# GadGadGad/Convolutional-KAN-for-Image-Classification

Measured on AMD Instinct MI355X. Metric: images/sec fwd+bwd KAN-VGG11 3x32x32 bs=256/GPU, higher is better.
Workload: dtype f32

## Files before the change

### convolutional-kan-for-image-classification_amd/_lib.py

```python
from __future__ import annotations

import ctypes as C
import os
from typing import Optional

_HERE = os.path.dirname(os.path.abspath(__file__))
LIB_PATH = os.environ.get("KANCONV_LIB") or os.path.join(_HERE, "libkanconv.so")

KAN_MAX_PLANES = 16
KAN_MAX_TABLE = 32
KAN_FP_WORDS = 192
BASIS_BSPLINE, BASIS_RBF, BASIS_CHEBY, BASIS_POLY, BASIS_FOURIER, BASIS_RELU, BASIS_GRAM = 0, 1, 2, 3, 4, 5, 6
ACT_NONE, ACT_IDENTITY, ACT_GELU, ACT_SILU, ACT_RELU, ACT_TANH, ACT_SIGMOID, ACT_GELU_TANH = -1, 0, 1, 2, 3, 4, 5, 6
ORDER_QUAD_FWD, ORDER_ROWBLK8_FWD, ORDER_QUAD_BWD_DATA, ORDER_FWD_WEIGHT_SIDE, ORDER_POS8_BWD_DATA = 1, 2, 4, 8, 16


class KanGeom(C.Structure):
    _fields_ = [(n, C.c_int) for n in ("B", "C", "H", "W", "O", "Ho", "Wo", "kh", "kw", "sh", "sw", "ph", "pw", "dh", "dw", "groups")] + \
               [("x_bstride", C.c_longlong), ("y_bstride", C.c_longlong)]


class KanBasis(C.Structure):
    _fields_ = [("kind", C.c_int), ("n_basis", C.c_int), ("order", C.c_int), ("act", C.c_int),
                ("p0", C.c_float), ("p1", C.c_float), ("table", C.c_float * KAN_MAX_TABLE), ("chan_table", C.c_void_p)]


class KanPlan(C.Structure):
    _fields_ = [(n, C.c_int) for n in ("P", "K", "IPC", "KC", "Kpad", "Opad", "fwd_splits", "bwd_data_splits", "bwd_weight_splits",
                                          "fwd_target", "bwd_data_target", "bwd_weight_target", "x_pm_wanted", "dz_pm_wanted", "bwd_weight_expanded", "row_blocks", "e_pm_wanted", "fwd_expanded", "fwd_halo", "bwd_weight_halo",
                                          "fwd_band", "bwd_weight_band")] + \
               [(n, C.c_longlong) for n in ("packed_weight_bytes", "bwd_data_weight_bytes", "fwd_slab_elems", "bwd_data_slab_elems",
                                            "bwd_weight_slab_elems", "e_pm_elems")]


class KanNormRoute(C.Structure):
    _fields_ = [(n, C.c_int) for n in ("kernel", "G", "EPL", "PPI", "NT", "pool", "lds", "held", "blocks", "strided")]

# ... 6 lines not shown
    _fields_ = [(n, C.c_int) for n in ("B", "C", "H", "W", "O", "Ho", "Wo", "kh", "kw", "sh", "sw", "ph", "pw", "dh", "dw", "wavelet")] + \
               [("x_bstride", C.c_longlong), ("u_bstride", C.c_longlong)]


class KanWavRoute(C.Structure):
    _fields_ = [(n, C.c_int) for n in ("TH", "TW", "NIMG", "RH", "RW", "tiles_h", "tiles_w", "fwd_shrunk", "fwd_nimg_cut", "fwd_lds_bytes", "fwd_fits",
                                       "fwd_blocks", "bwd_input_kernel", "bwd_input_blocks", "params_kernel", "passes", "chunks", "BH", "NI", "RU",
                                       "CU", "XP", "UP", "bands", "items", "items_per_chunk", "lds_bytes", "px_per_chunk")]


WAV_BI_TAPS9, WAV_BI_STRIDE1, WAV_BI_STRIDED = 0, 1, 2
WAV_PAR_TILED, WAV_PAR_PIXEL = 0, 1


WAVELETS = {"mexican_hat": 0, "morlet": 1, "dog": 2, "meyer": 3, "shannon": 4}

_P, _I, _LL, _F, _D = C.c_void_p, C.c_int, C.c_longlong, C.c_float, C.c_double
_GP, _BP = C.POINTER(KanGeom), C.POINTER(KanBasis)
SIGNATURES = {
    "kan_version": (C.c_char_p, []),
    "kan_last_error": (C.c_char_p, []),
    "kan_plan": (_I, [_GP, _BP, C.POINTER(KanPlan)]),
    "kan_tile_orders": (_I, [_GP, _BP]),
    "kan_pack_weights": (_I, [_P, _P, _P, _P, _GP, _BP, _P]),
    "kan_pack_weights_iod": (_I, [_P, _P, _P, _GP, _BP, _P]),
    "kan_pack_cacheable": (_I, [_GP, _BP]),
    "kan_pack_weights_cached": (_I, [_P, _P, _P, _P, _GP, _BP, _P, _I, _I, _I, _P]),
    "kan_conv_fwd": (_I, [_P, _P, _P, _P, _GP, _BP, _P, _P]),
    "kan_position_major": (_I, [_P, _P, _I, _I, _I, _LL, _P]),
    "kan_conv_bwd_data": (_I, [_P, _P, _P, _P, _P, _P, _GP, _BP, _P, _P]),
    "kan_conv_bwd_data_params": (_I, [_P, _P, _P, _P, _P, _P, _P, _GP, _BP, _P, _P]),
    "kan_conv_bwd_weight": (_I, [_P, _P, _P, _P, _GP, _BP, _P, _P, _P]),
    "kan_position_major_expanded": (_I, [_P, _P, _GP, _BP, _P]),
    "kan_conv_fwd_expanded": (_I, [_P, _P, _P, _GP, _BP, _P]),
    "kan_conv_fwd_expanded_order": (_I, [_P, _P, _P, _GP, _BP, _P, _I]),
    "kan_conv_bwd_weight_expanded": (_I, [_P, _P, _P, _GP, _BP, _P]),
    "kan_unpack_wgrad": (_I, [_P, _P, _P, _GP, _BP, _P]),
    "kan_unpack_wgrad_iod": (_I, [_P, _P, _GP, _BP, _P]),
    "kan_slab_reduce": (_I, [_P, _I, _LL, _P, _I, _I, _I, _LL, _P]),
    "kan_instnorm_prelu_fwd": (_I, [_P, _I, _LL, _P, _P, _P, _P, _P, _P, _P, _I, _I, _I, _LL, _F, _I, _P]),
    "kan_instnorm_prelu_bwd": (_I, [_P, _P, _P, _P, _P, _P, _P, _P, _P, _P, _P, _I, _I, _I, _LL, _I, _P]),
    "kan_instnorm_prelu_pool_fwd": (_I, [_P, _I, _LL, _P, _P, _P, _P, _P, _P, _P, _P, _I, _I, _I, _I, _LL, _F, _I, _P]),
    "kan_instnorm_prelu_pool_bwd": (_I, [_P, _P, _P, _P, _P, _P, _P, _P, _P, _P, _P, _P, _I, _I, _I, _I, _LL, _I, _P]),
    "kan_instnorm_prelu_poolk_fwd": (_I, [_P, _I, _LL, _P, _P, _P, _P, _P, _P, _P, _P, _I, _I, _I, _I, _LL, _F, _I, _I, _I, _P]),
    "kan_instnorm_prelu_poolk_bwd": (_I, [_P, _P, _P, _P, _P, _P, _P, _P, _P, _P, _P, _P, _I, _I, _I, _I, _LL, _I, _I, _I, _P]),
    "kan_norm_route": (_I, [_I, _I, _I, _I, _I, _LL, _I, _LL, _I, _I, _I, _I, C.POINTER(KanNormRoute)]),
# ... 75 lines not shown
```

### convolutional-kan-for-image-classification_amd/csrc/kan_internal.h

```cpp
#pragma once
#include <type_traits>
#include "kanconv.h"

int kan_fail_msg(const char* fmt, const char* a);
int kan_raise_lds_limit(const void* kernel, int bytes);

enum : int {
    FAST_GENERIC = 0,
    FAST_BSPLINE_SILU = 1,
    FAST_BSPLINE_GELU = 2,
    FAST_RBF8 = 3,
    FAST_CHEBY5 = 4,
    FAST_CHEBY4 = 5,
    FAST_POLY4 = 6,
    FAST_POLY3 = 7,
    FAST_RBF5 = 8,
    FAST_RELU8 = 9,
    FAST_GRAM4 = 10,
    FAST_POLY1 = 11,
    FAST_LAST = 11
};
enum : unsigned {
    ON_TAP_MAJOR = 1u << 0,
    ON_BIG_TILES = 1u << 1,
// ... 85 lines not shown
                               const KanBandCfg* cfg, int splits, long long slab_elems, void* stream);
int kan_band_fwd_launch(const float* x, const float* xn, const float* wp, float* z, const KanGeom* g, const KanBasis* b,
                        const KanBandCfg* cfg, int splits, long long slab_elems, void* stream);

constexpr int DW_T = 9;
constexpr int DW_MAX_TP = 96;

enum class Route { TAP_MAJOR, DW, BAND, HALO, EXPANDED };

struct FwdCfg { int TO, TP, tiles_o, tiles_p, chunks, splits, slots; };
struct BdCfg { int CH, tiles_c, tiles_p, n_ob, Opad32, chunks, splits; };
struct BwCfg { int TR, TO, tiles_r, tiles_o, chunks, splits, slots; };
struct BwHaloCfg { int R, nimg, spb, n_bands, tiles_r, tiles_o, splits, bands_per_split; };

struct ConvPlan {
    KanPlan pub;
    int fast;
    Route fwd, bwd_data, bwd_weight;
    bool pm_fwd, pm_bwd_data, pm_bwd_weight;
    bool rowblk_bwd_data;
    bool quad_fwd;
    bool quad_bd;
    bool pos8_bd;
    bool rowblk8_fwd;
    bool fwd_wq;
    bool pmdma_xcd, pm_lpt, pm_xcd;
    FwdCfg fc;
    BdCfg bd;
    BwCfg bw;
    BwHaloCfg bwh;
    KanBandCfg band;
};
int plan_conv(const KanGeom* g, const KanBasis* b, ConvPlan* cp);

int live_taps_out(const KanGeom* g, int hw);
int live_taps_in(const KanGeom* g, int hw);
int live_positions_for_tap(const KanGeom* g, int tap);
int balance_tiles(const int* weight, int n, unsigned short* idx);
```

### convolutional-kan-for-image-classification_amd/csrc/kan_plan.hip

```cpp
#include <hip/hip_runtime.h>
#include <cstdio>
#include <cstdlib>
#include <cstring>
#include "kanconv.h"
#include "kan_device.h"
#include "kan_common.h"
#include "kan_internal.h"

namespace {

int fail(const char* msg) { return kan_fail_msg("%s", msg); }

int check(const KanGeom* g, const KanBasis* b) {
    if (!g || !b) return fail("null geometry/basis");
    if (g->groups < 0 || g->groups > 65535) return fail("groups out of range");
    if (g->B <= 0 || g->C <= 0 || g->O <= 0 || g->H <= 0 || g->W <= 0 || g->Ho <= 0 || g->Wo <= 0) return fail("non-positive dimension");
    if (g->kh <= 0 || g->kw <= 0 || g->sh <= 0 || g->sw <= 0 || g->dh <= 0 || g->dw <= 0 || g->ph < 0 || g->pw < 0) return fail("bad conv parameters");
    if (g->kh > 255 || g->kw > 255 || g->C > 65535) return fail("kernel size / channel count out of supported range");
    if ((g->H + 2 * g->ph - g->dh * (g->kh - 1) - 1) / g->sh + 1 != g->Ho || (g->W + 2 * g->pw - g->dw * (g->kw - 1) - 1) / g->sw + 1 != g->Wo)
        return fail("Ho/Wo inconsistent with H/W, kernel, stride, padding, dilation");
    if ((long long)g->B * g->Ho * g->Wo >= (1ll << 31) || (long long)g->B * g->H * g->W >= (1ll << 31)) return fail("pixel count exceeds int32");
    if ((long long)g->B * g->x_bstride * 4 >= (1ll << 31) || (long long)g->B * g->y_bstride * 4 >= (1ll << 31))
        return fail("activation tensors must be smaller than 2 GiB (32-bit buffer offsets)");
    if (g->x_bstride < (long long)ngroups(g) * g->C * g->H * g->W || g->y_bstride < (long long)ngroups(g) * g->O * g->Ho * g->Wo)
// ... 179 lines not shown
}
BwHaloCfg bw_halo_cfg(const KanGeom* g, const KanPlan& pl) {
    BwHaloCfg c;
    c.R = g->W == 16 ? 4 : g->W;
    c.nimg = g->W == 4 ? 2 : 1;
    c.spb = c.nimg * c.R * g->W / 16;
    c.n_bands = g->B * (g->H / c.R) / c.nimg;
    c.tiles_r = ceil_div(pl.K, 128);
    c.tiles_o = pl.Opad / 128;
    const long long tiles = (long long)c.tiles_r * c.tiles_o * ngroups(g);
    const double slab_bytes = 4.0 * pl.K * pl.Opad * ngroups(g);
    int best = 1; double best_cost = -1;
    for (int sp = 1; sp <= c.n_bands && sp <= 1024; ++sp) {
        const int bps = ceil_div(c.n_bands, sp);
        if (ceil_div(c.n_bands, bps) != sp) continue;
        const long long rounds = (tiles * sp + 1023) / 1024;
        const double cost = (double)(rounds * (bps * c.spb + 6)) + sp * slab_cost_steps(slab_bytes);
        if (best_cost < 0 || cost < best_cost) { best_cost = cost; best = sp; }
    }
    c.splits = best;
    c.bands_per_split = ceil_div(c.n_bands, best);
    return c;
}
BwCfg bw_cfg(const KanGeom* g, const KanPlan& pl, bool big, bool pm_bw) {
    BwCfg c;
    c.TO = (big && !pm_bw) ? 256 : (pl.Opad % 128 == 0) ? 128 : 64;
    c.slots = c.TO == 256 ? 512 : 1024;
    c.TR = c.TO == 64 ? 256 : 128;
    c.tiles_r = ceil_div(pl.K, c.TR);
    c.tiles_o = pl.Opad / c.TO;
    c.chunks = ceil_div((long long)g->B * g->Ho * g->Wo, 16);
    c.splits = pick_splits((long long)c.tiles_r * c.tiles_o * ngroups(g), c.chunks, 16, 4.0 * pl.K * pl.Opad * ngroups(g), c.slots);
    return c;
}

bool dw_direct(const KanGeom* g, const KanBasis* b) {
    const bool off = tuning_off("KAN_DW");
    const int T = g->kh * g->kw, P = b->n_basis + (b->act != KAN_ACT_NONE);
    return !off && g->C == 1 && g->O <= 2 && T <= DW_T && T * P <= DW_MAX_TP;
}
int dw_weight_chunks(const KanGeom* g) {
    const long long total = (long long)g->B * g->Ho * g->Wo;
    int s = ceil_div(2048, ngroups(g));
    const int most = ceil_div(total, 256);
    if (s > most) s = most;
    if (s > 64) s = 64;
// ... 49 lines not shown
    for (int i = 0; i < n; ++i) { if (idx[i] >= n || seen[idx[i]]) return 0; seen[idx[i]] = true; }
    return n;
}

int plan_conv(const KanGeom* g, const KanBasis* b, ConvPlan* cp) {
    if (int rc = check(g, b)) return rc;
    ConvPlan& c = *cp;
    KanPlan* pl = &c.pub;
    const int T = g->kh * g->kw, G = ngroups(g), f = fast_variant(b);
    c.fast = f;
    const bool pm_shape = pmdma_fwd_shape(g, f);
    c.pm_fwd = want_pix_major(g, b, PM_FWD, pm_shape);
    c.pm_bwd_data = want_pix_major(g, b, PM_BWD_DATA, false);
    const bool want_pm_bw = want_pix_major(g, b, PM_BWD_WEIGHT, false);
    const bool dw = dw_direct(g, b);
    const bool halo = halo_fwd(g, b, f, c.pm_fwd);
    c.band.ok = c.band.bw_ok = 0;
    const bool band = band_fwd(g, b, f, dw, c.pm_fwd, halo, &c.band);
    const bool pmdma_fwd = pm_shape && c.pm_fwd;
    const bool pmdma_bw = pmdma_bwd_weight(g, b, f, want_pm_bw);
    const bool halo_bw = halo_bwd_weight(g, f, pmdma_bw);
    c.pm_bwd_weight = want_pm_bw && !halo_bw;
    const bool band_bw = band && c.band.bw_ok && !want_pm_bw && !tuning_off("KAN_BAND_BW");
    c.rowblk_bwd_data = rowblk_bwd_data(g, f, c.pm_bwd_data);
    c.pmdma_xcd = tuning_on("KAN_PMDMA_XCD");
    c.pm_lpt = !tuning_off("KAN_PM_LPT");
    c.pm_xcd = !tuning_off("KAN_PM_XCD");
    c.fwd = dw ? Route::DW : band ? Route::BAND : halo ? Route::HALO : pmdma_fwd ? Route::EXPANDED : Route::TAP_MAJOR;
    c.bwd_data = dw ? Route::DW : Route::TAP_MAJOR;
    c.bwd_weight = dw ? Route::DW : band_bw ? Route::BAND : halo_bw ? Route::HALO : pmdma_bw ? Route::EXPANDED : Route::TAP_MAJOR;
    pl->P = b->n_basis + (b->act != KAN_ACT_NONE);
    pl->K = g->C * T * pl->P;
    {
        int i18 = 18 / pl->P, i16 = 16 / pl->P;
        if (i18 > 4) i18 = 4;
        if (i16 > 4) i16 = 4;
        const bool use18 = (long long)i18 * pl->P * 16 > (long long)i16 * pl->P * 18;
        pl->KC = use18 ? 18 : 16;
        pl->IPC = use18 ? i18 : i16;
        if (pl->P >= 10 && pl->P <= 12) { pl->KC = 12; pl->IPC = 1; }
        if (halo) { pl->KC = 2 * pl->P; pl->IPC = 2; }
    }
    pl->Kpad = ceil_div(g->C * T, pl->IPC) * pl->KC;
    if (band) { pl->KC = c.band.NPLE; pl->IPC = c.band.NG; pl->Kpad = c.band.n_steps * c.band.NPLE; }
    pl->Opad = round_up(g->O, 64);
    pl->packed_weight_bytes = (long long)G * pl->Kpad * pl->Opad * 4;
// ... 64 lines not shown
```

### convolutional-kan-for-image-classification_amd/csrc/kanconv.hip

```cpp
#include <hip/hip_runtime.h>
#include <cstdio>
#include <cstdlib>
#include <cstring>
#include <cmath>
#include <cstdint>
#include <mutex>
#include <type_traits>
#include <vector>
#include "kanconv.h"
#include "kan_device.h"

#include "kan_common.h"
#include "kan_internal.h"

namespace {


thread_local char g_err[512] = "";
int fail(const char* fmt, const char* a = "") {
    snprintf(g_err, sizeof(g_err), fmt, a);
    return -1;
}
}
int kan_fail_msg(const char* fmt, const char* a) { return fail(fmt, a); }
// ... 1557 lines not shown
                acc[0][0] = MFMA32(fa[c_][0], fb[c_][0], acc[0][0]);
                acc[0][1] = MFMA32(fa[c_][0], fb[c_][1], acc[0][1]);
                acc[1][0] = MFMA32(fa[c_][1], fb[c_][0], acc[1][0]);
                acc[1][1] = MFMA32(fa[c_][1], fb[c_][1], acc[1][1]);
            }
#undef KAN_OFFA
#undef KAN_OFFB
        }
    }

    float* out = dwp + (size_t)blk.z * slab_elems;
#pragma unroll
    for (int mi = 0; mi < 2; ++mi)
#pragma unroll
        for (int r = 0; r < 16; ++r) {
            const int row = k0 + w_r * 64 + mi * 32 + mfma_row(r, lane);
            if (row >= Krows) continue;
#pragma unroll
            for (int ni = 0; ni < 2; ++ni) {
                const int o = o_tile0 + w_c * 64 + ni * 32 + (lane & 31);
                out[(size_t)row * Opad + o] = acc[mi][ni][r];
            }
        }
}

template <int KIND, int FAST>
__global__ __launch_bounds__(256) void k_expand_pm(const float* __restrict__ x, float* __restrict__ e_pm, DevBasis bs, int B, int CHW, int HW, int Cg,
                                                   long long bstride, float* __restrict__ dump) {
    __shared__ float tile[32][33];
    __shared__ float sTab[KAN_MAX_TABLE];
    const int e0 = blockIdx.x * 32, b0 = blockIdx.y * 32;
    const int tx = threadIdx.x & 31, ty = threadIdx.x >> 5;
    const int P = FAST ? fast_planes(FAST) : bs.P;
    if (threadIdx.x < KAN_MAX_TABLE) sTab[threadIdx.x] = bs.tab[threadIdx.x];
#pragma unroll
    for (int i = 0; i < 4; ++i) {
        const int b = b0 + ty + 8 * i, e = e0 + tx;
        tile[ty + 8 * i][tx] = (b < B && e < CHW) ? x[(size_t)b * bstride + e] : 0.f;
    }
    __syncthreads();
#pragma unroll
    for (int i = 0; i < 4; ++i) {
        const int e = e0 + ty + 8 * i, b = b0 + tx;
        if (e < CHW && b < B) {
            const float v = tile[tx][ty + 8 * i];
            stage_unit<KIND, FAST>(bs, sTab, true, v, v, e_pm + (size_t)e * P * B + b, B, dump + threadIdx.x, (e / HW) % Cg);
// ... 1246 lines not shown
        const int bx = c.tiles_c * 4, by = c.Opad32 / 32 * G;
        const long long nt = (long long)bx * by;
        const long long capd = fp ? 128 : 1024;
        dim3 gd((unsigned)(nt < capd ? nt : capd), 1, T);
        hipLaunchKernelGGL(k_pack_bwd_data, gd, dim3(256), 0, st, (const float*)wp, wd, q, c.CH, c.tiles_c, c.Opad32, wp_gs, bx, by, fp, fp_cur);
    }
    return launch_ok("pack");
}

int kan_pack_weights(const float* w_base, const float* w_basis, float* wp, float* wd, const KanGeom* g, const KanBasis* b, void* stream) {
    return pack_weights_impl(w_base, w_basis, wp, wd, g, b, nullptr, 0, stream);
}

int kan_pack_weights_iod(const float* coeffs, float* wp, float* wd, const KanGeom* g, const KanBasis* b, void* stream) {
    if (int rc = iod_scope(g, b)) return rc;
    return pack_weights_impl(nullptr, coeffs, wp, wd, g, b, nullptr, 0, stream, true);
}

int kan_tile_orders(const KanGeom* g, const KanBasis* b) {
    ConvPlan cp;
    if (plan_conv(g, b, &cp)) return 0;
    const bool halo = cp.fwd == Route::HALO;
    return (halo && cp.quad_fwd ? KAN_ORDER_QUAD_FWD : 0) | (halo && cp.rowblk8_fwd ? KAN_ORDER_ROWBLK8_FWD : 0) | (cp.quad_bd ? KAN_ORDER_QUAD_BWD_DATA : 0) |
           (cp.fwd_wq ? KAN_ORDER_FWD_WEIGHT_SIDE : 0) | (cp.pos8_bd ? KAN_ORDER_POS8_BWD_DATA : 0);
}

int kan_pack_cacheable(const KanGeom* g, const KanBasis* b) {
    ConvPlan cp;
    if (plan_conv(g, b, &cp)) return 0;
    if ((long long)g->O * g->C * (b->n_basis + 1) * g->kh * g->kw >= (1ll << 31)) return 0;
    return (!pack_needs_clear(g, cp.pub) && cp.fwd != Route::DW && ngroups(g) == 1) ? 1 : 0;
}

int kan_pack_weights_cached(const float* w_base, const float* w_basis, float* wp, float* wd, const KanGeom* g, const KanBasis* b,
                            unsigned long long* ring, int cur, int force, int sample_stride, void* stream) {
    static_assert(KAN_FP_WORDS == 3 * FP_LANES, "ring size");
    if (!ring || cur < 0 || cur > 2 || sample_stride < 1) return fail("bad fingerprint ring arguments");
    if (!kan_pack_cacheable(g, b)) return fail("cached packing is not offered for this geometry (kan_pack_cacheable)");
    const int hb = b->act != KAN_ACT_NONE;
    if ((hb && !w_base) || !w_basis) return fail("null weight pointer");
    if (((size_t)w_basis & 15) || (hb && ((size_t)w_base & 15))) return fail("cached packing needs 16-byte aligned weight tensors");
    const int T = g->kh * g->kw;
    const long long na = hb ? (long long)g->O * g->C * T : 0, nbs = (long long)g->O * g->C * b->n_basis * T;
    const long long groups4 = ((na + 3) / 4 + (nbs + 3) / 4 + sample_stride - 1) / sample_stride;
    long long blocks = (groups4 + 256 * 8 - 1) / (256 * 8); if (blocks > 4096) blocks = 4096; if (blocks < 1) blocks = 1;
    hipLaunchKernelGGL(k_fingerprint, dim3((unsigned)blocks), dim3(256), 0, (hipStream_t)stream, hb ? w_base : w_basis, (unsigned)na, w_basis,
                       (unsigned)nbs, (unsigned)sample_stride, ring, cur);
    if (int rc = launch_ok("fingerprint")) return rc;
    return pack_weights_impl(w_base, w_basis, wp, wd, g, b, force ? nullptr : ring, cur, stream);
}

static int unpack_wgrad_impl(const float* dwp, float* dw_base, float* dw_basis, const KanGeom* g, const KanBasis* b, void* stream, bool iod) {
    ConvPlan cp;
    if (int rc = plan_conv(g, b, &cp)) return rc;
    const KanPlan& pl = cp.pub;
    const int hb = b->act != KAN_ACT_NONE;
    if ((hb && !dw_base) || !dw_basis || !dwp) return fail("null weight-gradient pointer");
    hipStream_t st = (hipStream_t)stream;
    const int T = g->kh * g->kw, G = ngroups(g);
    const long long dwp_gs = (long long)(pl.bwd_weight_band ? pl.Kpad : pl.K) * pl.Opad;
    PackGeo q = pack_geo(g, b, cp, true);
    int n_slabs = pl.bwd_weight_splits;
    if (n_slabs >= 32) {
        hipLaunchKernelGGL(k_fold_slabs, dim3(ceil_div(pl.bwd_weight_slab_elems, 64)), dim3(256), 0, st, const_cast<float*>(dwp), n_slabs,
                           pl.bwd_weight_slab_elems, pl.bwd_weight_slab_elems);
        n_slabs = 1;
    }
    const int nb_base = hb ? ceil_div(g->C * T, UNPACK_TJ) : 0;
    dim3 grid(nb_base + ceil_div(g->C * b->n_basis * T, UNPACK_TJ), ceil_div(g->O, UNPACK_TO), G);
    if (iod) {
        const IodLaunch l = iod_launch(g, pl);
        hipLaunchKernelGGL(k_unpack_iod, dim3(l.blocks), dim3(256), 0, st, dwp, dw_basis, q, l.o_tiles, l.n_tiles, n_slabs, pl.bwd_weight_slab_elems,
                           iod_vec(dw_basis, dwp, g, b));
    } else {
        hipLaunchKernelGGL(k_unpack, grid, dim3(256), 0, st, dwp, dw_base, dw_basis, q, nb_base, n_slabs, pl.bwd_weight_slab_elems, dwp_gs);
    }
    return launch_ok("unpack");
}

int kan_unpack_wgrad(const float* dwp, float* dw_base, float* dw_basis, const KanGeom* g, const KanBasis* b, void* stream) {
    return unpack_wgrad_impl(dwp, dw_base, dw_basis, g, b, stream, false);
}

int kan_unpack_wgrad_iod(const float* dwp, float* dcoeffs, const KanGeom* g, const KanBasis* b, void* stream) {
    if (int rc = iod_scope(g, b)) return rc;
    return unpack_wgrad_impl(dwp, nullptr, dcoeffs, g, b, stream, true);
}

int kan_position_major(const float* src, float* dst, int B, int Cn, int HW, long long bstride, void* stream) {
    if (!src || !dst || B < 1 || Cn < 1 || HW < 1) return fail("bad position_major arguments");
    dim3 grid(ceil_div((long long)Cn * HW, 32), ceil_div(B, 32));
    hipLaunchKernelGGL(k_position_major, grid, dim3(256), 0, (hipStream_t)stream, src, dst, B, Cn * HW, bstride);
    return launch_ok("position_major");
}

int kan_conv_fwd(const float* x, const float* xn, const float* wp, float* z, const KanGeom* g, const KanBasis* b, const float* x_pm,
                 void* stream) {
    ConvPlan cp;
    if (int rc = plan_conv(g, b, &cp)) return rc;
    const KanPlan& pl = cp.pub;
    if (!x || !xn || !wp || !z) return fail("null tensor pointer");
    if ((b->kind == KAN_BASIS_RELU || b->kind == KAN_BASIS_GRAM) && !b->chan_table) return fail("ReLU / Gram bases need their device parameter table (chan_table)");
    hipStream_t st = (hipStream_t)stream;
    if (cp.fwd == Route::DW) {
// ... 198 lines not shown
    const int cps = dg.pix_major ? pl.bwd_weight_target : ceil_div(c.chunks, pl.bwd_weight_splits);
    if (x != xn && !fast_spec(cp.fast).xn_fwd)
        return fail("this basis / activation pair runs on single-input kernels: pass xn == x");
    auto launch = [&](auto kind, auto fast, auto wr, auto wc) {
        constexpr int WR = decltype(wr)::value, WC = decltype(wc)::value;
        hipLaunchKernelGGL((k_conv_bwd_weight<decltype(kind)::value, decltype(fast)::value, WR, WC>), grid, dim3(WR * WC * 64), 0, st, dz, x, xn, dwp,
                           dg, db, pl.K, pl.Opad, c.chunks, cps, pl.bwd_weight_slab_elems, x_bytes, dz_bytes, c.tiles_o);
    };
    auto tiles = [&](auto kind, auto fast) {
        if (c.TO == 128) launch(kind, fast, IC<2>{}, IC<2>{});
        else launch(kind, fast, IC<4>{}, IC<1>{});
    };
    const bool fast = dispatch_fast<ON_TAP_MAJOR>(cp.fast, [&](auto fv) {
        constexpr int F = decltype(fv)::value;
        if constexpr (fast_has(F, ON_BIG_TILES)) {
            if (c.TO == 256) return launch(IC<fast_kind(F)>{}, fv, IC<2>{}, IC<4>{});
        }
        tiles(IC<fast_kind(F)>{}, fv);
    });
    if (!fast) dispatch_kind(b->kind, [&](auto kind) { tiles(kind, IC<FAST_GENERIC>{}); });
    return launch_ok("conv_bwd_weight");
}

int kan_position_major_expanded(const float* x, float* e_pm, const KanGeom* g, const KanBasis* b, void* stream) {
    ConvPlan cp;
    if (int rc = plan_conv(g, b, &cp)) return rc;
    const KanPlan& pl = cp.pub;
    if (!x || !e_pm) return fail("null tensor pointer");
    if (!pl.e_pm_wanted) return fail("this geometry / basis does not use the expanded position-major copy (plan.e_pm_wanted)");
    const int G = ngroups(g), CHW = G * g->C * g->H * g->W;
    DevBasis db = dev_basis(b);
    dim3 grid(ceil_div(CHW, 32), ceil_div(g->B, 32));
    float* dump = e_pm + (pl.e_pm_elems - 256);
    if ((b->kind == KAN_BASIS_RELU || b->kind == KAN_BASIS_GRAM) && !b->chan_table) return fail("ReLU / Gram bases need their device parameter table (chan_table)");
    dispatch_fast<ON_EXPANDED>(cp.fast, [&](auto fv) {
        constexpr int F = decltype(fv)::value;
        hipLaunchKernelGGL((k_expand_pm<fast_kind(F), F>), grid, dim3(256), 0, (hipStream_t)stream, x, e_pm, db, g->B, CHW, g->H * g->W, g->C, g->x_bstride, dump);
    });
    return launch_ok("position_major_expanded");
}

static int conv_fwd_expanded_impl(const float* e_pm, const float* wp, float* z, const KanGeom* g, const KanBasis* b, void* stream, int order) {
    ConvPlan cp;
    if (int rc = plan_conv(g, b, &cp)) return rc;
    const KanPlan& pl = cp.pub;
    if (!e_pm || !wp || !z) return fail("null tensor pointer");
// ... 303 lines not shown
```

### convolutional-kan-for-image-classification_amd/ops.py

```python
from __future__ import annotations

import contextlib
import ctypes as C
import os
import weakref
from collections import OrderedDict
from dataclasses import dataclass, replace
from functools import lru_cache, partial, wraps
from typing import List, NamedTuple, Optional, Sequence, Tuple

import torch
from torch.autograd.function import once_differentiable

from . import _lib as L


@dataclass(frozen=True)
class ConvSpec:
    kind: int
    n_basis: int
    order: int
    act: int
    p0: float
    p1: float
# ... 36 lines not shown
        raise L.KanConvError(f"basis table of {len(spec.table)} entries exceeds KAN_MAX_TABLE={L.KAN_MAX_TABLE}")
    for i, v in enumerate(spec.table):
        b.table[i] = v
    return b


@lru_cache(maxsize=512)
def _plan_cached(spec: ConvSpec, B: int, Cg: int, H: int, W: int, Og: int, C_total: int, O_total: int):
    Ho, Wo = spec.out_hw(H, W)
    if Ho <= 0 or Wo <= 0:
        raise L.KanConvError(f"empty output ({Ho}x{Wo}) for input {H}x{W}")
    g = L.KanGeom()
    g.B, g.C, g.H, g.W, g.O, g.Ho, g.Wo = B, Cg, H, W, Og, Ho, Wo
    (g.kh, g.kw), (g.sh, g.sw), (g.ph, g.pw), (g.dh, g.dw) = spec.kernel, spec.stride, spec.padding, spec.dilation
    g.x_bstride, g.y_bstride = C_total * H * W, O_total * Ho * Wo
    g.groups = spec.groups
    b = _basis_struct(spec)
    p = L.KanPlan()
    bp = b
    if _device_table(spec):
        bp = L.KanBasis.from_buffer_copy(b)
        bp.chan_table = 1
    L.check(L.load().kan_plan(C.byref(g), C.byref(bp), C.byref(p)), "kan_plan")
    p.tile_orders = L.load().kan_tile_orders(C.byref(g), C.byref(bp))
    return g, b, p


def _plan_key(spec: ConvSpec, shape, Og: int) -> tuple:
    B, Ct, H, W = shape
    return (spec, B, Ct // spec.groups, H, W, Og, Ct, Og * spec.groups)


def _with_phases(basis: L.KanBasis, phases: Optional[torch.Tensor], mode: int = 0) -> L.KanBasis:
    if phases is None:
        return basis
    b = L.KanBasis.from_buffer_copy(basis)
    b.chan_table, b.order = phases.data_ptr(), mode
    return b


_TABLES: "dict[tuple, torch.Tensor]" = {}


def _with_table(basis: L.KanBasis, spec: ConvSpec, device) -> L.KanBasis:
    if not _device_table(spec):
        return basis
# ... 77 lines not shown
                for t in range(kw):
                    hi, wi = ho * sh - ph + r * dh, wo * sw - pw + t * dw
                    live += 0 <= hi < H and 0 <= wi < W
    return live / float(Ho * Wo * kh * kw)


_ROW_BLOCK_BIT = {"fwd": 1, "bwd_data": 2, "bwd_weight": 0}


def _quadrant_order(geom, plan, which: str) -> bool:
    return which == "fwd" and bool(plan.row_blocks & 1) and geom.B % 32 == 0


def _quadrant_bwd_data(geom, plan, have_dz_pm: bool) -> bool:
    return bool(have_dz_pm) and bool(plan.row_blocks & 2) and bool(getattr(plan, "tile_orders", 0) & L.ORDER_QUAD_BWD_DATA)


def _row_blocks8_forward(geom, plan) -> bool:
    return geom.H == 8 and geom.W == 8 and bool(getattr(plan, "tile_orders", 0) & L.ORDER_ROWBLK8_FWD)


def _pos8_bwd_data(geom, plan) -> bool:
    return bool(getattr(plan, "tile_orders", 0) & L.ORDER_POS8_BWD_DATA)


def _executed_flops(geom, plan, which: str, have_dz_pm: bool = False) -> float:
    target = {"fwd": plan.fwd_target, "bwd_data": plan.bwd_data_target, "bwd_weight": plan.bwd_weight_target}[which]
    dense = _conv_flops(geom, plan)
    g = geom
    if target <= 0:
        if _quadrant_order(geom, plan, which) or (which == "bwd_data" and _quadrant_bwd_data(geom, plan, have_dz_pm)):
            return dense * _live_fraction(which, g.H, g.W, g.Ho, g.Wo, g.kh, g.kw, g.sh, g.sw, g.ph, g.pw, g.dh, g.dw)
        if plan.row_blocks & _ROW_BLOCK_BIT[which]:
            return dense * (5.0 / 6.0)
        if which == "fwd" and _row_blocks8_forward(geom, plan):
            return dense * (11.0 / 12.0)
        if which == "bwd_data" and have_dz_pm and _pos8_bwd_data(geom, plan):
            return dense * (484.0 / 576.0)
        return dense
    return dense * _live_fraction(which, g.H, g.W, g.Ho, g.Wo, g.kh, g.kw, g.sh, g.sw, g.ph, g.pw, g.dh, g.dw)


def _layer_tag(geom) -> str:
    return f"{geom.C * max(1, geom.groups)}->{geom.O * max(1, geom.groups)}@{geom.H}x{geom.W} k{geom.kh}x{geom.kw}"


# ... 402 lines not shown
    Cg = Ct // G
    Ot = dz.shape[1]
    Og = Ot // G
    geom, basis, plan = _plan_cached(*_plan_key(spec, x.shape, Og))
    basis = _with_table(_with_phases(basis, phases, mode), spec, x.device)
    kh, kw = spec.kernel
    st = _stream(x)
    xs = xn if xn is not None else x
    wd, x_pm = packed
    dw_base: List[Optional[torch.Tensor]] = [None] * G
    dw_basis: List[Optional[torch.Tensor]] = [None] * G
    split_w = need_w and dw_split
    split_x = need_x and wcd is not None
    exact_w = need_w and not split_w
    exact_x = (need_x or need_xn) and not split_x
    dz_pm = _position_major(dz, 0, Ot) if (xn is None and ((plan.dz_pm_wanted and (exact_w or exact_x)) or (exact_x and _pos8_bwd_data(geom, plan)))) else None
    if split_w:
        sb, ss = (_sink_for(wids[0], (Og, Cg, kh, kw), x.device), _sink_for(wids[1], (Og, Cg * spec.n_basis, kh, kw), x.device)) if wids else (None, None)
        dwb = sb if sb is not None else torch.empty((Og, Cg, kh, kw), device=x.device, dtype=torch.float32)
        dws = ss if ss is not None else torch.empty((Og, Cg * spec.n_basis, kh, kw), device=x.device, dtype=torch.float32)
        kan_conv_bwd_weight_split(spec, x, dz, out=(dwb, dws))
        dw_base, dw_basis = list(dwb.unsqueeze(0).unbind(0)), list(dws.unsqueeze(0).unbind(0))
    elif exact_w:
        dwp = torch.empty(plan.bwd_weight_splits * plan.bwd_weight_slab_elems, device=x.device, dtype=torch.float32)
        if plan.bwd_weight_expanded and xn is None and dz_pm is not None:
            e_pm = x_pm if (plan.fwd_expanded and not plan.x_pm_wanted and x_pm is not None and mode == 0) else _expand_pm(x, geom, basis, plan, st)
            _launch(_sample("bwd_weight", geom, plan, True, expanded=True), x,
                    lambda: lib.kan_conv_bwd_weight_expanded(_ptr(dz_pm), _ptr(e_pm), _ptr(dwp), C.byref(geom), C.byref(basis), st))
        else:
            _launch(_sample("bwd_weight", geom, plan, x_pm is not None and dz_pm is not None, xn is not None), x,
                    lambda: lib.kan_conv_bwd_weight(_ptr(dz), _ptr(x), _ptr(xs), _ptr(dwp), C.byref(geom), C.byref(basis), _ptr(x_pm),
                                                    _ptr(dz_pm), st))
        if spec.w_layout == W_IOD:
            dco = torch.empty((Cg, Og, spec.n_basis), device=x.device, dtype=torch.float32)
            L.check(lib.kan_unpack_wgrad_iod(_ptr(dwp), _ptr(dco), C.byref(geom), C.byref(basis), st), "kan_unpack_wgrad_iod")
            dw_basis = [dco]
        else:
            sb = _sink_for(wids[0], (Og, Cg, kh, kw), x.device) if (wids and G == 1 and spec.has_base) else None
            ss = _sink_for(wids[1], (Og, Cg * spec.n_basis, kh, kw), x.device) if (wids and G == 1) else None
            dwb = (sb.unsqueeze(0) if sb is not None else
                   torch.empty((G, Og, Cg, kh, kw), device=x.device, dtype=torch.float32)) if spec.has_base else None
            dws = ss.unsqueeze(0) if ss is not None else torch.empty((G, Og, Cg * spec.n_basis, kh, kw), device=x.device, dtype=torch.float32)
            L.check(lib.kan_unpack_wgrad(_ptr(dwp), _ptr(dwb), _ptr(dws), C.byref(geom), C.byref(basis), st), "kan_unpack_wgrad")
            dw_basis = list(dws.unbind(0))
            if spec.has_base:
                dw_base = list(dwb.unbind(0))
    dx = dxn = None
    if split_x:
        dx, _ = kan_conv_bwd_data_split(spec, x, dz, None, None, wcd)
    elif exact_x:
        S = plan.bwd_data_splits
        separate = xn is not None
        dxs = torch.empty((S, B, Ct, H, W), device=x.device, dtype=torch.float32)
        dxns = torch.empty_like(dxs) if separate else None
        head, tail = (_ptr(dz), _ptr(x), _ptr(xs), _ptr(wd), _ptr(dxs), _ptr(dxns)), (C.byref(geom), C.byref(basis), _ptr(dz_pm), st)
        _launch(_sample("bwd_data", geom, plan, dz_pm is not None), x,
                (lambda: lib.kan_conv_bwd_data(*head, *tail)) if dparams is None else
                (lambda: lib.kan_conv_bwd_data_params(*head, _ptr(dparams), *tail)))
        dx, dxn = _sum_slabs(dxs, B, Ct, H * W), (_sum_slabs(dxns, B, Ct, H * W) if separate else None)
    return dx, dxn, dw_base, dw_basis


def _sum_slabs(slabs: torch.Tensor, B: int, Cn: int, HW: int) -> torch.Tensor:
    if slabs.shape[0] == 1:
        return slabs[0]
    out = torch.empty_like(slabs[0])
# ... 585 lines not shown
```

### include/kanconv.h

```cpp
#ifndef KANCONV_H
#define KANCONV_H

#ifdef __cplusplus
extern "C" {
#endif

#define KAN_MAX_PLANES 16
#define KAN_MAX_TABLE  32
#define KAN_FP_WORDS   192

enum { KAN_BASIS_BSPLINE = 0, KAN_BASIS_RBF = 1, KAN_BASIS_CHEBY = 2, KAN_BASIS_POLY = 3, KAN_BASIS_FOURIER = 4, KAN_BASIS_RELU = 5, KAN_BASIS_GRAM = 6 };
enum { KAN_ACT_NONE = -1, KAN_ACT_IDENTITY = 0, KAN_ACT_GELU = 1, KAN_ACT_SILU = 2, KAN_ACT_RELU = 3,
       KAN_ACT_TANH = 4, KAN_ACT_SIGMOID = 5, KAN_ACT_GELU_TANH = 6 };

typedef struct KanGeom {
    int B, C, H, W;
    int O, Ho, Wo;
    int kh, kw, sh, sw, ph, pw, dh, dw;
    int groups;
    long long x_bstride;
    long long y_bstride;
} KanGeom;

#define KAN_ORDER_PACK(mode, first) ((int)(mode) | ((int)(first) << 8))
// ... 19 lines not shown
    int bwd_weight_expanded;
    int row_blocks;
    int e_pm_wanted, fwd_expanded;
    int fwd_halo, bwd_weight_halo;
    int fwd_band, bwd_weight_band;
    long long packed_weight_bytes;
    long long bwd_data_weight_bytes;
    long long fwd_slab_elems;
    long long bwd_data_slab_elems;
    long long bwd_weight_slab_elems;
    long long e_pm_elems;
} KanPlan;

const char* kan_version(void);
const char* kan_last_error(void);

int kan_plan(const KanGeom* geom, const KanBasis* basis, KanPlan* plan);

#define KAN_ORDER_QUAD_FWD 1
#define KAN_ORDER_ROWBLK8_FWD 2
#define KAN_ORDER_QUAD_BWD_DATA 4
#define KAN_ORDER_FWD_WEIGHT_SIDE 8
#define KAN_ORDER_POS8_BWD_DATA 16
int kan_tile_orders(const KanGeom* geom, const KanBasis* basis);

int kan_pack_weights(const float* w_base, const float* w_basis, float* wp, float* wd,
                     const KanGeom* geom, const KanBasis* basis, void* stream);

int kan_pack_weights_iod(const float* coeffs, float* wp, float* wd, const KanGeom* geom, const KanBasis* basis, void* stream);

int kan_pack_cacheable(const KanGeom* geom, const KanBasis* basis);
int kan_pack_weights_cached(const float* w_base, const float* w_basis, float* wp, float* wd,
                            const KanGeom* geom, const KanBasis* basis, unsigned long long* ring, int cur, int force,
                            int sample_stride, void* stream);

int kan_conv_fwd(const float* x, const float* xn, const float* wp, float* z,
                 const KanGeom* geom, const KanBasis* basis, const float* x_pm, void* stream);

int kan_position_major(const float* src, float* dst, int B, int Cn, int HW, long long bstride, void* stream);

int kan_conv_bwd_data(const float* dz, const float* x, const float* xn, const float* wd,
                      float* dx, float* dxn,
                      const KanGeom* geom, const KanBasis* basis, const float* dz_pm, void* stream);

int kan_conv_bwd_data_params(const float* dz, const float* x, const float* xn, const float* wd, float* dx, float* dxn, float* dparams,
                             const KanGeom* geom, const KanBasis* basis, const float* dz_pm, void* stream);

int kan_conv_bwd_weight(const float* dz, const float* x, const float* xn, float* dwp,
                        const KanGeom* geom, const KanBasis* basis, const float* x_pm, const float* dz_pm, void* stream);

int kan_position_major_expanded(const float* x, float* e_pm, const KanGeom* geom, const KanBasis* basis, void* stream);
int kan_conv_fwd_expanded(const float* e_pm, const float* wp, float* z, const KanGeom* geom, const KanBasis* basis, void* stream);
int kan_conv_fwd_expanded_order(const float* e_pm, const float* wp, float* z, const KanGeom* geom, const KanBasis* basis, void* stream, int order);
int kan_conv_bwd_weight_expanded(const float* dz_pm, const float* e_pm, float* dwp,
                                 const KanGeom* geom, const KanBasis* basis, void* stream);

int kan_unpack_wgrad(const float* dwp, float* dw_base, float* dw_basis,
                     const KanGeom* geom, const KanBasis* basis, void* stream);

int kan_unpack_wgrad_iod(const float* dwp, float* dcoeffs, const KanGeom* geom, const KanBasis* basis, void* stream);

int kan_slab_reduce(const float* slabs, int n_slabs, long long slab_elems, float* out,
                    int B, int Cn, int HW, long long bstride, void* stream);

int kan_instnorm_prelu_fwd(const float* z, int n_slabs, long long slab_elems, float* z_out,
                           const float* gamma, const float* beta, const float* prelu_a,
                           float* y, float* mean, float* rstd,
                           int B, int Cn, int HW, long long bstride, float eps, int prelu_span, void* stream);

int kan_instnorm_prelu_bwd(const float* dy, const float* z, const float* mean, const float* rstd,
                           const float* gamma, const float* beta, const float* prelu_a,
                           float* dz, float* dgamma, float* dbeta, float* dprelu,
                           int B, int Cn, int HW, long long bstride, int prelu_span, void* stream);

int kan_instnorm_prelu_pool_fwd(const float* z, int n_slabs, long long slab_elems, float* z_out,
                                const float* gamma, const float* beta, const float* prelu_a,
                                float* y_pooled, unsigned char* pool_idx, float* mean, float* rstd,
                                int B, int Cn, int H, int W, long long bstride, float eps, int prelu_span, void* stream);
// ... 137 lines not shown
```

Measured before the change: 18230.

## Add 8x8 tap-skipping weight-gradient kernel for B-spline KAN convs

Adds a specialized backward-weight kernel for 8x8 3x3 stride-1 B-spline layers. It stages the expanded input halo and dz rows in LDS, and uses hand-scheduled LDS reads with MFMA that skip the padding taps at the image edges. Split count comes from a cost model, and a matching unpack path handles the new slab layout. The aim is to cut wasted MFMA work and memory traffic on the small deep VGG layers. The price is more LDS use, inline asm, and a separate code path.

```diff
diff --git a/convolutional-kan-for-image-classification_amd/_lib.py b/convolutional-kan-for-image-classification_amd/_lib.py
--- a/convolutional-kan-for-image-classification_amd/_lib.py
+++ b/convolutional-kan-for-image-classification_amd/_lib.py
@@ -13,6 +13,7 @@
 BASIS_BSPLINE, BASIS_RBF, BASIS_CHEBY, BASIS_POLY, BASIS_FOURIER, BASIS_RELU, BASIS_GRAM = 0, 1, 2, 3, 4, 5, 6
 ACT_NONE, ACT_IDENTITY, ACT_GELU, ACT_SILU, ACT_RELU, ACT_TANH, ACT_SIGMOID, ACT_GELU_TANH = -1, 0, 1, 2, 3, 4, 5, 6
 ORDER_QUAD_FWD, ORDER_ROWBLK8_FWD, ORDER_QUAD_BWD_DATA, ORDER_FWD_WEIGHT_SIDE, ORDER_POS8_BWD_DATA = 1, 2, 4, 8, 16
+ORDER_POS8_BWD_WEIGHT = 32
 
 
 class KanGeom(C.Structure):
@@ -65,6 +66,9 @@
     "kan_last_error": (C.c_char_p, []),
     "kan_plan": (_I, [_GP, _BP, C.POINTER(KanPlan)]),
     "kan_tile_orders": (_I, [_GP, _BP]),
+    "kan_bwd_weight_rowgroup_slabs": (_I, [_GP, _BP]),
+    "kan_conv_bwd_weight_rowgroups": (_I, [_P, _P, _P, _GP, _BP, _P]),
+    "kan_unpack_wgrad_rowgroups": (_I, [_P, _P, _P, _GP, _BP, _P]),
     "kan_pack_weights": (_I, [_P, _P, _P, _P, _GP, _BP, _P]),
     "kan_pack_weights_iod": (_I, [_P, _P, _P, _GP, _BP, _P]),
     "kan_pack_cacheable": (_I, [_GP, _BP]),
diff --git a/convolutional-kan-for-image-classification_amd/csrc/kan_internal.h b/convolutional-kan-for-image-classification_amd/csrc/kan_internal.h
--- a/convolutional-kan-for-image-classification_amd/csrc/kan_internal.h
+++ b/convolutional-kan-for-image-classification_amd/csrc/kan_internal.h
@@ -131,6 +131,7 @@
     bool quad_fwd;
     bool quad_bd;
     bool pos8_bd;
+    bool pos8_bw;
     bool rowblk8_fwd;
     bool fwd_wq;
     bool pmdma_xcd, pm_lpt, pm_xcd;
@@ -138,6 +139,7 @@
     BdCfg bd;
     BwCfg bw;
     BwHaloCfg bwh;
+    BwHaloCfg p8;
     KanBandCfg band;
 };
 int plan_conv(const KanGeom* g, const KanBasis* b, ConvPlan* cp);
diff --git a/convolutional-kan-for-image-classification_amd/csrc/kan_plan.hip b/convolutional-kan-for-image-classification_amd/csrc/kan_plan.hip
--- a/convolutional-kan-for-image-classification_amd/csrc/kan_plan.hip
+++ b/convolutional-kan-for-image-classification_amd/csrc/kan_plan.hip
@@ -225,6 +225,34 @@
     c.bands_per_split = ceil_div(c.n_bands, best);
     return c;
 }
+bool pos8_bw_cfg(const KanGeom* g, int f, bool dw, BwHaloCfg* out) {
+    if (tuning_off("KAN_POS8_BW") || !fast_has(f, ON_HALO_BWD_WEIGHT) || fast_kind(f) != KAN_BASIS_BSPLINE || dw) return false;
+    if (g->H != 8 || g->W != 8 || g->Ho != 8 || g->Wo != 8 || g->kh != 3 || g->kw != 3 || g->sh != 1 || g->sw != 1 || g->ph != 1 || g->pw != 1 ||
+        g->dh != 1 || g->dw != 1) return false;
+    if (g->B % 2 != 0 || g->C > 65535 / 81) return false;
+    if ((long long)g->B * g->x_bstride * 4 >= (1ll << 31) || (long long)g->B * g->y_bstride * 4 >= (1ll << 31)) return false;
+    BwHaloCfg c;
+    const int P = fast_planes(f), Opad = round_up(g->O, 64);
+    c.R = 8; c.nimg = 2; c.spb = 8;
+    c.n_bands = g->B / 2;
+    c.tiles_r = ceil_div(g->C * P, 32);
+    c.tiles_o = ceil_div(Opad, 128);
+    const long long tiles = (long long)c.tiles_r * c.tiles_o * ngroups(g);
+    const double slab_bytes = 4.0 * g->C * 9 * P * Opad * ngroups(g);
+    int best = 1; double best_cost = -1;
+    for (int sp = 1; sp <= c.n_bands && sp <= 1024; ++sp) {
+        const int bps = ceil_div(c.n_bands, sp);
+        if (ceil_div(c.n_bands, bps) != sp || (bps < 2 && c.n_bands >= 2)) continue;
+        const long long rounds = (tiles * sp + 511) / 512;
+        const double cost = (double)(rounds * (bps * c.spb * 2 + 6)) + sp * slab_cost_steps(slab_bytes);
+        if (best_cost < 0 || cost < best_cost) { best_cost = cost; best = sp; }
+    }
+    c.splits = best;
+    c.bands_per_split = ceil_div(c.n_bands, best);
+    if (c.n_bands > 8 && tiles * c.splits < 256) return false;
+    *out = c;
+    return true;
+}
 BwCfg bw_cfg(const KanGeom* g, const KanPlan& pl, bool big, bool pm_bw) {
     BwCfg c;
     c.TO = (big && !pm_bw) ? 256 : (pl.Opad % 128 == 0) ? 128 : 64;
@@ -320,6 +348,7 @@
     const bool halo_bw = halo_bwd_weight(g, f, pmdma_bw);
     c.pm_bwd_weight = want_pm_bw && !halo_bw;
     const bool band_bw = band && c.band.bw_ok && !want_pm_bw && !tuning_off("KAN_BAND_BW");
+    c.pos8_bw = pos8_bw_cfg(g, f, dw, &c.p8);
     c.rowblk_bwd_data = rowblk_bwd_data(g, f, c.pm_bwd_data);
     c.pmdma_xcd = tuning_on("KAN_PMDMA_XCD");
     c.pm_lpt = !tuning_off("KAN_PM_LPT");
diff --git a/convolutional-kan-for-image-classification_amd/csrc/kanconv.hip b/convolutional-kan-for-image-classification_amd/csrc/kanconv.hip
--- a/convolutional-kan-for-image-classification_amd/csrc/kanconv.hip
+++ b/convolutional-kan-for-image-classification_amd/csrc/kanconv.hip
@@ -1603,6 +1603,174 @@
                 out[(size_t)row * Opad + o] = acc[mi][ni][r];
             }
         }
+}
+
+#define P8_READ(dst, addr, off) asm volatile("ds_read_b32 %0, %1 offset:%2" : "=&v"(dst) : "v"(addr), "n"(off) : "memory")
+#define P8_WAIT(reg, N) asm volatile("s_waitcnt lgkmcnt(%1)" : "+v"(reg) : "n"(N) : "memory")
+#define P8_TIE(reg) asm volatile("" : "+v"(reg))
+constexpr int P8_W = 8, P8_HWC = P8_W + 2, P8_HIMG = P8_HWC * P8_HWC, P8_CELLS = 2 * P8_HIMG;
+constexpr int P8_PS = P8_CELLS + 1;
+constexpr int P8_NCH = 5, P8_ZB = 16 * 128;
+__host__ __device__ constexpr bool pos8_col_live(int w, int t) { return w + t - 1 >= 0 && w + t - 1 < P8_W; }
+__host__ __device__ constexpr int pos8_col_reads(int w, int rows) { return 1 + rows * ((w == 0 || w == P8_W - 1) ? 2 : 3); }
+
+template <int RK, int ZPAR>
+__device__ __forceinline__ void pos8_row(f32x16 (&acc)[9], unsigned a_row, const unsigned (&bB)[8]) {
+    constexpr int R0 = RK == 0 ? 1 : 0, R1 = RK == 2 ? 1 : 2, NR = R1 - R0 + 1;
+    float fa[2][9], fb[2];
+#define P8_READS(w_, s_)                                                                                                          \
+    do {                                                                                                                         \
+        P8_READ(fb[s_], bB[w_], ZPAR * P8_ZB * 4);                                                                              \
+        _Pragma("unroll") for (int r = R0; r <= R1; ++r)                                                                         \
+            _Pragma("unroll") for (int t = 0; t < 3; ++t)                                                                        \
+                if (pos8_col_live(w_, t)) P8_READ(fa[s_][r * 3 + t], a_row, (r * P8_HWC + t + (w_)) * 4);                        \
+    } while (0)
+    P8_READS(0, 0);
+#pragma unroll
+    for (int w = 0; w < P8_W; ++w) {
+        const int c_ = w & 1, n_ = c_ ^ 1;
+        if (w + 1 < P8_W) {
+            P8_READS(w + 1, n_);
+            P8_WAIT(fb[c_], pos8_col_reads(w + 1 < P8_W ? w + 1 : 0, NR));
+        } else {
+            P8_WAIT(fb[c_], 0);
+        }
+#pragma unroll
+        for (int r = R0; r <= R1; ++r)
+#pragma unroll
+            for (int t = 0; t < 3; ++t)
+                if (pos8_col_live(w, t)) {
+                    P8_TIE(fa[c_][r * 3 + t]);
+                    acc[r * 3 + t] = MFMA32(fa[c_][r * 3 + t], fb[c_], acc[r * 3 + t]);
+                }
+    }
+#undef P8_READS
+}
+
+template <int FAST>
+__global__ __launch_bounds__(256, 2) void k_conv_bwd_weight_pos8(
+    const float* __restrict__ dz, const float* __restrict__ x, float* __restrict__ dwp, DevGeom g, DevBasis bs, int Krows, int Opad,
+    int n_bands, int bands_per_split, long long slab_elems, unsigned x_bytes, unsigned dz_bytes, int tiles_o) {
+    constexpr int KIND = fast_kind(FAST);
+    constexpr int P = fast_planes(FAST), T = 9, NT = 256;
+    constexpr int HB = P8_NCH * P * P8_PS;
+    constexpr int NU = P8_NCH * 2 * P8_W * P8_W;
+    constexpr int SLOTS = (NU + NT - 1) / NT;
+    static_assert(P == 9, "row groups of 32 (c, p) pairs: nine planes per channel");
+    __shared__ float sH[HB];
+    __shared__ __attribute__((aligned(16))) float sZ[2 * P8_ZB];
+    __shared__ float sTab[KAN_MAX_TABLE];
+
+    const int tid = threadIdx.x, lane = tid & 63;
+    const int wave = __builtin_amdgcn_readfirstlane(tid >> 6);
+    const int kh2 = lane >> 5;
+    const BlockId blk = xcd_block_order(true);
+    const int grp = blk.y / tiles_o;
+    const int q0 = blk.x * 32, o_tile0 = (blk.y - grp * tiles_o) * 128;
+    x += (size_t)grp * g.C * 64;
+    dz += (size_t)grp * g.O * 64;
+    dwp += (size_t)grp * Krows * Opad;
+    const int c0 = q0 / P;
+
+    if (tid < KAN_MAX_TABLE) sTab[tid] = bs.tab[tid];
+    for (int i = tid; i < HB; i += NT) sH[i] = 0.f;
+    float* const dump = sH + P8_CELLS;
+
+    int u_src[SLOTS], u_dst[SLOTS], u_ch[SLOTS]; unsigned u_ok = 0;
+#pragma unroll
+    for (int k = 0; k < SLOTS; ++k) {
+        const int idx = tid + k * NT;
+        const int ch = idx >> 7, img = (idx >> 6) & 1, pos = idx & 63, h = pos >> 3, w = pos & 7;
+        u_src[k] = (c0 + ch) * 64 + img * (int)g.xbs + pos;
+        u_dst[k] = ch * (P * P8_PS) + img * P8_HIMG + (h + 1) * P8_HWC + w + 1;
+        u_ch[k] = c0 + ch;
+        u_ok |= ((idx < NU && c0 + ch < g.C) ? 1u : 0u) << k;
+    }
+    const kan_rsrc x_rs = make_rsrc(x, x_bytes), dz_rs = make_rsrc(dz, dz_bytes);
+
+    const unsigned aA = lds_addr(sH + (q0 + (lane & 31) - c0 * P) * P8_PS + kh2 * P8_HIMG);
+    unsigned bB[8];
+    {
+        const int ol = wave * 32 + (lane & 31), sw = (ol >> 1) & 15;
+#pragma unroll
+        for (int kk = 0; kk < 8; ++kk) bB[kk] = lds_addr(sZ + ol * 16 + ((2 * kk + kh2) ^ sw));
+    }
+    unsigned zoff[8];
+#pragma unroll
+    for (int j = 0; j < 8; ++j) {
+        const int ol = 4 * (wave * 8 + j) + (lane >> 4), q = (lane & 15) ^ ((ol >> 1) & 15);
+        zoff[j] = o_tile0 + ol < g.O ? (unsigned)((o_tile0 + ol) * 64 + (q >> 1) + (q & 1) * (int)g.ybs) * 4u : KAN_OOB;
+    }
+    auto issue_dz = [&](int band, int st, int zb) {
+        const int soff = __builtin_amdgcn_readfirstlane((2 * band * (int)g.ybs + st * P8_W) * 4);
+        float* dst = sZ + zb * P8_ZB + wave * (8 * 64);
+#pragma unroll
+        for (int j = 0; j < 8; ++j)
+            __builtin_amdgcn_raw_ptr_buffer_load_lds(dz_rs, (__attribute__((address_space(3))) void*)(dst + j * 64), 4, (int)zoff[j], soff, 0, 0);
+    };
+    float xv[SLOTS];
+    auto load_band = [&](int band) {
+        const int sbase = 2 * band * (int)g.xbs;
+#pragma unroll
+        for (int k = 0; k < SLOTS; ++k) xv[k] = buf_load(x_rs, ((u_ok >> k) & 1u) ? (unsigned)(sbase + u_src[k]) * 4u : KAN_OOB);
+    };
+    auto expand_band = [&]() {
+#pragma unroll
+        for (int k = 0; k < SLOTS; ++k)
+            if ((u_ok >> k) & 1u) stage_unit<KIND, FAST>(bs, sTab, true, xv[k], xv[k], sH + u_dst[k], P8_PS, dump, u_ch[k]);
+    };
+
+    f32x16 acc[9];
+#pragma unroll
+    for (int a = 0; a < 9; ++a)
+#pragma unroll
+        for (int r = 0; r < 16; ++r) acc[a][r] = 0.f;
+
+    const int nb0 = blk.z * bands_per_split, nb1 = min(n_bands, nb0 + bands_per_split);
+    __syncthreads();
+    if (nb0 < nb1) {
+        load_band(nb0);
+        expand_band();
+        issue_dz(nb0, 0, 0);
+    }
+    for (int band = nb0; band < nb1; ++band) {
+        const bool more = band + 1 < nb1;
+        auto step = [&](int st) {
+            asm volatile("s_waitcnt vmcnt(0)" ::: "memory");
+            __syncthreads();
+            if (st + 1 < P8_W) issue_dz(band, st + 1, (st + 1) & 1);
+            else if (more) issue_dz(band + 1, 0, 0);
+            if (st == 0 && more) load_band(band + 1);
+        };
+        step(0);
+        pos8_row<0, 0>(acc, aA, bB);
+#pragma unroll 1
+        for (int st = 1; st < P8_W - 1; st += 2) {
+            step(st);
+            pos8_row<1, 1>(acc, aA + (unsigned)(st * P8_HWC * 4), bB);
+            step(st + 1);
+            pos8_row<1, 0>(acc, aA + (unsigned)((st + 1) * P8_HWC * 4), bB);
+        }
+        step(P8_W - 1);
+        pos8_row<2, 1>(acc, aA + (unsigned)((P8_W - 1) * P8_HWC * 4), bB);
+        if (more) {
+            __syncthreads();
+            expand_band();
+        }
+    }
+
+    float* out = dwp + (size_t)blk.z * slab_elems;
+    const int o = o_tile0 + wave * 32 + (lane & 31);
+    if (o < Opad) {
+#pragma unroll
+        for (int r = 0; r < 16; ++r) {
+            const int q = q0 + mfma_row(r, lane);
+            if (q >= g.C * P) continue;
+            const int c = q / P, p = q - c * P;
+#pragma unroll
+            for (int tap = 0; tap < T; ++tap) out[(size_t)((c * T + tap) * P + p) * Opad + o] = acc[tap][r];
+        }
+    }
 }
 
 template <int KIND, int FAST>
@@ -2895,7 +3063,8 @@
     if (plan_conv(g, b, &cp)) return 0;
     const bool halo = cp.fwd == Route::HALO;
     return (halo && cp.quad_fwd ? KAN_ORDER_QUAD_FWD : 0) | (halo && cp.rowblk8_fwd ? KAN_ORDER_ROWBLK8_FWD : 0) | (cp.quad_bd ? KAN_ORDER_QUAD_BWD_DATA : 0) |
-           (cp.fwd_wq ? KAN_ORDER_FWD_WEIGHT_SIDE : 0) | (cp.pos8_bd ? KAN_ORDER_POS8_BWD_DATA : 0);
+           (cp.fwd_wq ? KAN_ORDER_FWD_WEIGHT_SIDE : 0) | (cp.pos8_bd ? KAN_ORDER_POS8_BWD_DATA : 0) |
+           (cp.pos8_bw ? KAN_ORDER_POS8_BWD_WEIGHT : 0);
 }
 
 int kan_pack_cacheable(const KanGeom* g, const KanBasis* b) {
@@ -2923,9 +3092,16 @@
     return pack_weights_impl(w_base, w_basis, wp, wd, g, b, force ? nullptr : ring, cur, stream);
 }
 
-static int unpack_wgrad_impl(const float* dwp, float* dw_base, float* dw_basis, const KanGeom* g, const KanBasis* b, void* stream, bool iod) {
+static int unpack_wgrad_impl(const float* dwp, float* dw_base, float* dw_basis, const KanGeom* g, const KanBasis* b, void* stream, bool iod, bool pos8 = false) {
     ConvPlan cp;
     if (int rc = plan_conv(g, b, &cp)) return rc;
+    if (pos8) {
+        if (!cp.pos8_bw) return fail("this geometry / basis does not offer the 8x8 tap-skipping weight gradient (kan_tile_orders)");
+        cp.bwd_weight = Route::HALO;
+        cp.pub.bwd_weight_band = 0;
+        cp.pub.bwd_weight_splits = cp.p8.splits;
+        cp.pub.bwd_weight_slab_elems = (long long)ngroups(g) * cp.pub.K * cp.pub.Opad;
+    }
     const KanPlan& pl = cp.pub;
     const int hb = b->act != KAN_ACT_NONE;
     if ((hb && !dw_base) || !dw_basis || !dwp) return fail("null weight-gradient pointer");
@@ -2953,6 +3129,10 @@
 
 int kan_unpack_wgrad(const float* dwp, float* dw_base, float* dw_basis, const KanGeom* g, const KanBasis* b, void* stream) {
     return unpack_wgrad_impl(dwp, dw_base, dw_basis, g, b, stream, false);
+}
+
+int kan_unpack_wgrad_rowgroups(const float* dwp, float* dw_base, float* dw_basis, const KanGeom* g, const KanBasis* b, void* stream) {
+    return unpack_wgrad_impl(dwp, dw_base, dw_basis, g, b, stream, false, true);
 }
 
 int kan_unpack_wgrad_iod(const float* dwp, float* dcoeffs, const KanGeom* g, const KanBasis* b, void* stream) {
@@ -3197,6 +3377,33 @@
     return launch_ok("conv_bwd_weight");
 }
 
+int kan_bwd_weight_rowgroup_slabs(const KanGeom* g, const KanBasis* b) {
+    ConvPlan cp;
+    if (plan_conv(g, b, &cp)) return 0;
+    return cp.pos8_bw ? cp.p8.splits : 0;
+}
+
+int kan_conv_bwd_weight_rowgroups(const float* dz, const float* x, float* dwp, const KanGeom* g, const KanBasis* b, void* stream) {
+    ConvPlan cp;
+    if (int rc = plan_conv(g, b, &cp)) return rc;
+    const KanPlan& pl = cp.pub;
+    if (!dz || !x || !dwp) return fail("null tensor pointer");
+    if (!cp.pos8_bw) return fail("this geometry / basis does not offer the 8x8 tap-skipping weight gradient (kan_tile_orders)");
+    const BwHaloCfg& hc = cp.p8;
+    const DevGeom dgh = dev_geom(g); const DevBasis dbh = dev_basis(b);
+    if ((long long)hc.tiles_o * ngroups(g) > 65535) return fail("groups * output tiles exceed the grid limit");
+    const unsigned x_bytes = (unsigned)((long long)g->B * g->x_bstride * 4), dz_bytes = (unsigned)((long long)g->B * g->y_bstride * 4);
+    const long long slab_elems = (long long)ngroups(g) * pl.K * pl.Opad;
+    dim3 grid(hc.tiles_r, hc.tiles_o * ngroups(g), hc.splits);
+    dispatch_fast<ON_HALO_BWD_WEIGHT>(cp.fast, [&](auto fv) {
+        constexpr int F = decltype(fv)::value;
+        if constexpr (fast_kind(F) == KAN_BASIS_BSPLINE)
+            hipLaunchKernelGGL((k_conv_bwd_weight_pos8<F>), grid, dim3(256), 0, (hipStream_t)stream, dz, x, dwp, dgh, dbh, pl.K, pl.Opad, hc.n_bands,
+                               hc.bands_per_split, slab_elems, x_bytes, dz_bytes, hc.tiles_o);
+    });
+    return launch_ok("conv_bwd_weight_pos8");
+}
+
 int kan_position_major_expanded(const float* x, float* e_pm, const KanGeom* g, const KanBasis* b, void* stream) {
     ConvPlan cp;
     if (int rc = plan_conv(g, b, &cp)) return rc;
diff --git a/convolutional-kan-for-image-classification_amd/ops.py b/convolutional-kan-for-image-classification_amd/ops.py
--- a/convolutional-kan-for-image-classification_amd/ops.py
+++ b/convolutional-kan-for-image-classification_amd/ops.py
@@ -82,6 +82,7 @@
         bp = L.KanBasis.from_buffer_copy(b)
         bp.chan_table = 1
     L.check(L.load().kan_plan(C.byref(g), C.byref(bp), C.byref(p)), "kan_plan")
+    p.pos8_bw_slabs = L.load().kan_bwd_weight_rowgroup_slabs(C.byref(g), C.byref(bp))
     p.tile_orders = L.load().kan_tile_orders(C.byref(g), C.byref(bp))
     return g, b, p
 
@@ -205,6 +206,10 @@
 
 def _pos8_bwd_data(geom, plan) -> bool:
     return bool(getattr(plan, "tile_orders", 0) & L.ORDER_POS8_BWD_DATA)
+
+
+def _pos8_bwd_weight(geom, plan) -> bool:
+    return bool(getattr(plan, "tile_orders", 0) & L.ORDER_POS8_BWD_WEIGHT)
 
 
 def _executed_flops(geom, plan, which: str, have_dz_pm: bool = False) -> float:
@@ -653,8 +658,14 @@
         kan_conv_bwd_weight_split(spec, x, dz, out=(dwb, dws))
         dw_base, dw_basis = list(dwb.unsqueeze(0).unbind(0)), list(dws.unsqueeze(0).unbind(0))
     elif exact_w:
-        dwp = torch.empty(plan.bwd_weight_splits * plan.bwd_weight_slab_elems, device=x.device, dtype=torch.float32)
-        if plan.bwd_weight_expanded and xn is None and dz_pm is not None:
+        pos8 = xn is None and spec.w_layout != W_IOD and _pos8_bwd_weight(geom, plan)
+        slabs = plan.pos8_bw_slabs * G * plan.K * plan.Opad if pos8 else plan.bwd_weight_splits * plan.bwd_weight_slab_elems
+        dwp = torch.empty(slabs, device=x.device, dtype=torch.float32)
+        if pos8:
+            name, dense, _, tag = _sample("bwd_weight", geom, plan, False)
+            _launch(("k_conv_bwd_weight_pos8/" + name.split("/")[1], dense, dense * (484.0 / 576.0), tag), x,
+                    lambda: lib.kan_conv_bwd_weight_rowgroups(_ptr(dz), _ptr(x), _ptr(dwp), C.byref(geom), C.byref(basis), st))
+        elif plan.bwd_weight_expanded and xn is None and dz_pm is not None:
             e_pm = x_pm if (plan.fwd_expanded and not plan.x_pm_wanted and x_pm is not None and mode == 0) else _expand_pm(x, geom, basis, plan, st)
             _launch(_sample("bwd_weight", geom, plan, True, expanded=True), x,
                     lambda: lib.kan_conv_bwd_weight_expanded(_ptr(dz_pm), _ptr(e_pm), _ptr(dwp), C.byref(geom), C.byref(basis), st))
@@ -672,7 +683,8 @@
             dwb = (sb.unsqueeze(0) if sb is not None else
                    torch.empty((G, Og, Cg, kh, kw), device=x.device, dtype=torch.float32)) if spec.has_base else None
             dws = ss.unsqueeze(0) if ss is not None else torch.empty((G, Og, Cg * spec.n_basis, kh, kw), device=x.device, dtype=torch.float32)
-            L.check(lib.kan_unpack_wgrad(_ptr(dwp), _ptr(dwb), _ptr(dws), C.byref(geom), C.byref(basis), st), "kan_unpack_wgrad")
+            unpack = lib.kan_unpack_wgrad_rowgroups if pos8 else lib.kan_unpack_wgrad
+            L.check(unpack(_ptr(dwp), _ptr(dwb), _ptr(dws), C.byref(geom), C.byref(basis), st), "kan_unpack_wgrad")
             dw_basis = list(dws.unbind(0))
             if spec.has_base:
                 dw_base = list(dwb.unbind(0))
diff --git a/include/kanconv.h b/include/kanconv.h
--- a/include/kanconv.h
+++ b/include/kanconv.h
@@ -65,6 +65,7 @@
 #define KAN_ORDER_QUAD_BWD_DATA 4
 #define KAN_ORDER_FWD_WEIGHT_SIDE 8
 #define KAN_ORDER_POS8_BWD_DATA 16
+#define KAN_ORDER_POS8_BWD_WEIGHT 32
 int kan_tile_orders(const KanGeom* geom, const KanBasis* basis);
 
 int kan_pack_weights(const float* w_base, const float* w_basis, float* wp, float* wd,
@@ -97,6 +98,10 @@
 int kan_conv_fwd_expanded_order(const float* e_pm, const float* wp, float* z, const KanGeom* geom, const KanBasis* basis, void* stream, int order);
 int kan_conv_bwd_weight_expanded(const float* dz_pm, const float* e_pm, float* dwp,
                                  const KanGeom* geom, const KanBasis* basis, void* stream);
+
+int kan_bwd_weight_rowgroup_slabs(const KanGeom* geom, const KanBasis* basis);
+int kan_conv_bwd_weight_rowgroups(const float* dz, const float* x, float* dwp, const KanGeom* geom, const KanBasis* basis, void* stream);
+int kan_unpack_wgrad_rowgroups(const float* dwp, float* dw_base, float* dw_basis, const KanGeom* geom, const KanBasis* basis, void* stream);
 
 int kan_unpack_wgrad(const float* dwp, float* dw_base, float* dw_basis,
                      const KanGeom* geom, const KanBasis* basis, void* stream);
```

New measurement: 18550 (median of 6 runs). 1.02x the previous value.
